# tyb311/TCCT

Measured on AMD Instinct MI355X. Metric: OCT B-scans/sec fwd+bwd(+clip+AdamW), stc_tt bs=8 1x800x1100, higher is better.
Workload: dtype bf16; 1 GPU; stc_tt --los=di bs=8/GPU 1x800x1100 (net tensors 3x800x1104); global_batch=8, parallelism=dp1, ranks=1, grad_allreduce=none, slowest_step=136

## Files before the change

### tcct_amd/csrc/pw_mfma.hip

```cpp
#include "common.h"
#include "c3_geom.h"
#include <cstdlib>

typedef __attribute__((ext_vector_type(8))) __bf16 bf16x8;
typedef __attribute__((ext_vector_type(16))) float f32x16;
typedef __attribute__((ext_vector_type(4))) short s16x4;
typedef __attribute__((ext_vector_type(8))) short s16x8;

#define PWB 256

__device__ __forceinline__ void st_out4(bf16* p, float a, float b, float c, float d) {
    uint2 o; o.x = pack_bf16x2(a, b); o.y = pack_bf16x2(c, d);
    *reinterpret_cast<uint2*>(p) = o;
}
__device__ __forceinline__ void st_out4(float* p, float a, float b, float c, float d) {
    *reinterpret_cast<float4*>(p) = make_float4(a, b, c, d);
}


struct PwUp { const float* p; int uH, uW, Ho, Wo; float sh, sw; uint32_t m_howo, m_wo; };
struct PwSplit { const bf16* x2; int K1; void* y2; int N1; const bf16* res; const float* rscale; int64_t per_sample; bf16* yplain; C3Geom c3; PwUp up; };
template <int NT, typename Tout, bool STATS, bool AFF, bool C3 = false>
__global__ void __launch_bounds__(PWB, 2)
k_pw_fwd(const bf16* __restrict__ x, const float* __restrict__ w, const float* __restrict__ bias, Tout* __restrict__ y,
// ... 315 lines not shown
    const int64_t M = (int64_t)B * Ho * Wo;
    TCCT_CHECK(M < (1ll << 31), "pw_fwd_f32_upadd: %lld pixels exceed the 32-bit index arithmetic", (long long)M);
    PwSplit sp{nullptr, 0, nullptr, 0, nullptr, nullptr, 1, nullptr};
    sp.up = PwUp{up, uH, uW, Ho, Wo, Ho > 1 ? (float)(uH - 1) / (float)(Ho - 1) : 0.f, Wo > 1 ? (float)(uW - 1) / (float)(Wo - 1) : 0.f,
                 (uint32_t)((1ull << 32) / (uint64_t)(Ho * Wo)), (uint32_t)((1ull << 32) / (uint64_t)Wo)};
    return pw_fwd_impl(x, w, bias, y, M, K, N, 0, TCCT_F32, nullptr, 0, stream, nullptr, 0, 0, sp);
}
extern "C" int tcct_pw_dgrad_split2(const void* dy, const float* w, void* dx1, void* dx2, int K1, int64_t M, int Nout, int K,
                                    tcct_stream_t stream) {
    TCCT_CHECK(dx2 != nullptr, "pw_dgrad_split2: dx2 is NULL");
    return pw_fwd_impl(dy, w, nullptr, dx1, M, Nout, K, 1, TCCT_BF16, nullptr, 0, stream, nullptr, 0, 0, PwSplit{nullptr, 0, dx2, K1, nullptr, nullptr, 1, nullptr});
}
extern "C" int tcct_pw_fwd_residual(const void* x, const float* w, const float* bias, const void* res, const float* scale,
                                    int64_t per_sample, void* y, void* y_plain, int64_t M, int K, int N, tcct_stream_t stream) {
    TCCT_CHECK(res != nullptr && N % 32 == 0 && per_sample >= 1, "pw_fwd_residual: needs res, N %% 32 == 0, per_sample >= 1");
    return pw_fwd_impl(x, w, bias, y, M, K, N, 0, TCCT_BF16, nullptr, 0, stream, nullptr, 0, 0,
                       PwSplit{nullptr, 0, nullptr, 0, (const bf16*)res, scale, per_sample, (bf16*)y_plain});
}
extern "C" int tcct_pw_dgrad_residual(const void* dy, const float* w, const void* res, void* dx_sum, void* dx_plain, int64_t M, int Nout,
                                      int K, tcct_stream_t stream) {
    TCCT_CHECK(res != nullptr && K % 32 == 0, "pw_dgrad_residual: needs res, K %% 32 == 0");
    return pw_fwd_impl(dy, w, nullptr, dx_sum, M, Nout, K, 1, TCCT_BF16, nullptr, 0, stream, nullptr, 0, 0,
                       PwSplit{nullptr, 0, nullptr, 0, (const bf16*)res, nullptr, 1, (bf16*)dx_plain});
}
extern "C" int tcct_pw_fwd_affine(const void* x, const float* w, const float* bias, void* y, int64_t M, int K, int N, const float* ab,
                                  int pre_act, int post_act, int out_dtype, tcct_stream_t stream) {
    return pw_fwd_impl(x, w, bias, y, M, K, N, 0, out_dtype, nullptr, 0, stream, ab, pre_act, post_act);
}
extern "C" int tcct_pw_fwd_affine_residual(const void* x, const float* w, const float* bias, const float* ab, const void* res, void* y, int64_t M, int K, int N,
                                           tcct_stream_t stream) {
    TCCT_CHECK(res != nullptr && pw_fwd2_aff_ok(M, K, N, false, true), "pw_fwd_affine_residual: K=%d N=%d unsupported (64, 96 or 128 square) or res NULL", K, N);
    return pw_fwd2_launch(x, nullptr, w, bias, y, M, K, N, nullptr, 0, stream, pw_res_affine((const bf16*)res, nullptr, ab, TCCT_ACT_NONE));
}
extern "C" int tcct_pw_fwd_xaff_affine_residual(const void* y_prev, const float* ab_prev, const float* w, const float* bias, const float* ab, const void* res, void* y,
                                                int64_t M, int K, int N, tcct_stream_t stream) {
    TCCT_CHECK(y_prev && ab_prev && res != nullptr && pw_fwd2_aff_ok(M, K, N, false, true), "pw_fwd_xaff_affine_residual: K=%d N=%d unsupported (64, 96 or 128 square) or NULL argument", K, N);
    PwFwd2Mode md;
    md.xap = TCCT_ACT_HSWISH;
    return pw_fwd2_launch(y_prev, nullptr, w, bias, y, M, K, N, nullptr, 0, stream, pw_res_affine((const bf16*)res, ab_prev, ab, TCCT_ACT_NONE), md);
}
extern "C" int tcct_pw_fwd_cat2_affine(const void* x1, const void* x2, const float* w, const float* bias, const float* ab, int post_act, void* y, int64_t M, int K, int N,
                                       tcct_stream_t stream) {
    TCCT_CHECK(x2 != nullptr && pw_fwd2_aff_ok(M, K, N, true, false), "pw_fwd_cat2_affine: K=%d N=%d unsupported (64 + 64 -> 96)", K, N);
    return pw_fwd2_launch(x1, x2, w, bias, y, M, K, N, nullptr, 0, stream, pw_res_affine(nullptr, nullptr, ab, post_act));
}
static int pw_fwd_impl(const void* x, const float* w, const float* bias, void* y, int64_t M, int K, int N, int transposed,
                       int out_dtype, double* stats, int stat_pre, tcct_stream_t stream, const float* aff, int aff_pre, int aff_post, PwSplit sp) {
    if (!transposed && out_dtype == TCCT_BF16 && (aff || aff_post) && !aff_pre && !stats && !sp.y2 && !sp.yplain && !sp.rscale && pw_fwd2_enabled()
        && pw_fwd2_aff_ok(M, K, N, sp.x2 != nullptr, sp.res != nullptr) && (!sp.x2 || sp.K1 == 64))
        return pw_fwd2_launch(x, sp.x2, w, bias, y, M, K, N, nullptr, 0, stream, pw_res_affine(sp.res, nullptr, aff, aff_post));
    if (!transposed && out_dtype == TCCT_BF16 && !aff && !aff_pre && !aff_post && !sp.y2 && pw_fwd2_enabled()
        && pw_fwd2_ok(M, K, N, sp.K1, sp.x2 != nullptr) && (!stats || N <= 128) && !(sp.res && (sp.x2 || stats)))
        return pw_fwd2_launch(x, sp.x2, w, bias, y, M, K, N, stats, stat_pre, stream, pw_res_train(sp.res, sp.rscale, sp.per_sample, sp.yplain));
    if (sp.x2) TCCT_CHECK(sp.K1 % 32 == 0 && sp.K1 > 0 && sp.K1 < K, "pw_fwd_cat2: K1=%d must be a multiple of 32 inside (0, K)", sp.K1);
    if (sp.y2) TCCT_CHECK(sp.N1 % 32 == 0 && sp.N1 > 0 && sp.N1 < N && N % 32 == 0 && out_dtype == TCCT_BF16, "pw_dgrad_split2: N1=%d must be a multiple of 32 inside (0, N), bf16 output", sp.N1);
    TCCT_CHECK(K % 32 == 0 && K >= 32 && K <= 512, "pw_fwd: K=%d must be a multiple of 32 (<=512)", K);
    TCCT_CHECK(N >= 1 && N <= 1024, "pw_fwd: N=%d", N);
    const int ntiles = (N + 31) / 32;
    int NT = ntiles <= 5 ? ntiles : (ntiles % 5 == 0 ? 5 : (ntiles % 4 == 0 ? 4 : (ntiles % 3 == 0 ? 3 : (ntiles % 2 == 0 ? 2 : 1))));
    const int64_t mblocks = ((M + 31) / 32 + 3) / 4;
    while (NT > 1 && mblocks * ((ntiles + NT - 1) / NT) < 512) {
        int nn = NT - 1;
        while (nn > 1 && ntiles % nn != 0) --nn;
        NT = nn;
    }
    if (stats && NT > 4) NT = 1;
    const int gy = (ntiles + NT - 1) / NT;
    size_t lds = (((size_t)NT * 32 * (2 * K + 16) + 15) & ~(size_t)15) + 4 * 2560 + (size_t)NT * 32 * 4;
    TCCT_CHECK(lds <= 160 * 1024, "pw_fwd: weights need %zu B of LDS", lds);
    const int64_t mtiles = (M + 31) / 32;
    int64_t gx = (mtiles + 3) / 4;
    int per_cu = (int)((160 * 1024) / lds);
    if (per_cu > 4) per_cu = 4;
    if (per_cu < 1) per_cu = 1;
    const int cap = 256 * per_cu;
    if (gx > cap) gx = cap;
    hipStream_t st = (hipStream_t)stream;
#define PW_GO(NTV, TO, ST, AF) tcct_launch<k_pw_fwd<NTV, TO, ST, AF>, 160 * 1024>(dim3((unsigned)gx, gy), dim3(PWB), lds, st, (const bf16*)x, w, bias, (TO*)y, M, K, N, transposed, \
                                                                                stats, stats ? stat_pre : 0, aff, aff_pre, aff_post, sp)
#define PW_NT4(TO, ST, AF) case 1: PW_GO(1, TO, ST, AF); break; case 2: PW_GO(2, TO, ST, AF); break; case 3: PW_GO(3, TO, ST, AF); break; case 4: PW_GO(4, TO, ST, AF); break
    bool hit = true;
    if (aff || aff_pre || aff_post || sp.res) {
        TCCT_CHECK(out_dtype == TCCT_BF16 && !stats, "pw_fwd_affine: bf16 output only");
        switch (NT) { PW_NT4(bf16, false, true); case 5: PW_GO(5, bf16, false, true); break; default: hit = false; }
    }
    else if (stats) switch (NT) { PW_NT4(bf16, true, false); default: hit = false; }
    else if (out_dtype == TCCT_BF16) switch (NT) { PW_NT4(bf16, false, false); case 5: PW_GO(5, bf16, false, false); break; default: hit = false; }
    else if (out_dtype == TCCT_F32) switch (NT) { PW_NT4(float, false, false); case 5: PW_GO(5, float, false, false); break; default: hit = false; }
    else { tcct_set_error("pw_fwd: bad out dtype"); return -1; }
#undef PW_NT4
#undef PW_GO
    TCCT_CHECK(hit, "pw_fwd: no kernel for %d N-tiles per block (stats %d)", NT, stats != nullptr);
    TCCT_LAUNCH_OK();
}

extern "C" int tcct_c3_fwd(const void* x4, const float* w, const float* bias, void* y, int B, int H, int W, int stride, double* stats,
                           int stat_pre, const float* ab, int pre_act, int post_act, tcct_stream_t stream) {
    TCCT_CHECK(stride == 1 || stride == 2, "c3_fwd: stride %d", stride);
    TCCT_CHECK(!(stats && (ab || pre_act || post_act)), "c3_fwd: fused statistics and the inference epilogue exclude each other");
    TCCT_CHECK(!stats || stat_pre == 0, "c3_fwd: the fused statistics are those of the raw output (both first layers feed a BatchNorm directly)");
    const int Ho = (H - 1) / stride + 1, Wo = (W - 1) / stride + 1;
    const int64_t M = (int64_t)B * Ho * Wo, inb = (int64_t)B * H * W * 8;
    TCCT_CHECK(M > 0 && M < (1ll << 31) - 64 && inb < (1ll << 31), "c3_fwd: image too large for 32-bit pixel offsets (B=%d H=%d W=%d)", B, H, W);
    const int tpr = (Wo + 31) / 32;
    auto magic = [](uint32_t d) { return d == 1 ? 0xffffffffu : (uint32_t)((1ull << 32) / d); };
    PwSplit sp{nullptr, 0, nullptr, 0, nullptr, nullptr, 1, nullptr,
               C3Geom{H, W, Ho, Wo, stride, (uint32_t)inb, tpr, magic((uint32_t)tpr), magic((uint32_t)Ho), magic((uint32_t)(Ho * Wo)), magic((uint32_t)Wo)}};
    const size_t lds = (((size_t)32 * (2 * 48 + 16) + 15) & ~(size_t)15) + 4 * 2560 + 32 * 4;
    const int64_t mtiles = (int64_t)B * Ho * tpr;
    int64_t gx = (mtiles + 3) / 4;
    if (gx > 256 * 4) gx = 256 * 4;
    hipStream_t st = (hipStream_t)stream;
    if (stats)
        hipLaunchKernelGGL((k_pw_fwd<1, bf16, true, false, true>), dim3((unsigned)gx, 1), dim3(PWB), lds, st, (const bf16*)x4, w, bias, (bf16*)y, M, 48, 32, 0,
                           stats, stat_pre, nullptr, 0, 0, sp);
    else if (ab || pre_act || post_act)
        hipLaunchKernelGGL((k_pw_fwd<1, bf16, false, true, true>), dim3((unsigned)gx, 1), dim3(PWB), lds, st, (const bf16*)x4, w, bias, (bf16*)y, M, 48, 32, 0,
                           nullptr, 0, ab, pre_act, post_act, sp);
    else
        hipLaunchKernelGGL((k_pw_fwd<1, bf16, false, false, true>), dim3((unsigned)gx, 1), dim3(PWB), lds, st, (const bf16*)x4, w, bias, (bf16*)y, M, 48, 32, 0,
                           nullptr, 0, nullptr, 0, 0, sp);
    TCCT_LAUNCH_OK();
}

__device__ __forceinline__ bf16x8 tr_load8g(const unsigned char* base, int stride, int P, int chan0, int lane) {
    const int i = lane & 15, q = i >> 2, pp = i & 3, g = lane >> 4;
    const int hh = g >> 1, cb = g & 1;
    const unsigned char* a0 = base + (P + 8 * hh + q) * stride + (chan0 + 16 * cb + 4 * pp) * 2;
    s16x4 lo = __builtin_amdgcn_ds_read_tr16_b64_v4i16((__attribute__((address_space(3))) s16x4*)a0);
    s16x4 hi = __builtin_amdgcn_ds_read_tr16_b64_v4i16((__attribute__((address_space(3))) s16x4*)(a0 + 4 * stride));
    s16x8 v = __builtin_shufflevector(lo, hi, 0, 1, 2, 3, 4, 5, 6, 7);
    return __builtin_bit_cast(bf16x8, v);
}

#define PW_P 128
#define PW_XS 4
#define PW_DS 10
template <int NT, int KTB, bool C3 = false>
__global__ void __launch_bounds__(PWB, 2)
k_pw_wgrad(const bf16* __restrict__ x, const bf16* __restrict__ dy, float* __restrict__ dw, float* __restrict__ dbias, int64_t M,
           int K, int N, int SX, int SD, const bf16* __restrict__ x2, int K1, int64_t ldy, C3Geom g3 = C3Geom{0, 0, 0, 0, 0, 0u, 0, 0u, 0u, 0u, 0u}) {
    extern __shared__ __attribute__((aligned(16))) unsigned char smem[];
    unsigned char* sX = smem;
    unsigned char* sD = smem + PW_P * SX;
    const int tid = threadIdx.x, lane = tid & 63, wave = tid >> 6;
    const int r = lane & 31, hh = lane >> 5;
    const int ci_base = blockIdx.y * KTB * 32;
    const bf16* xsrc = (x2 && ci_base >= K1) ? x2 + (ci_base - K1) : x + ci_base;
    const int ldx = x2 ? (ci_base >= K1 ? K - K1 : K1) : K;
    const int xc = KTB * 4, dc = N >> 3;
    f32x16 acc[NT][KTB];
#pragma unroll
    for (int a = 0; a < NT; ++a)
#pragma unroll
        for (int b = 0; b < KTB; ++b)
#pragma unroll
            for (int k = 0; k < 16; ++k) acc[a][b][k] = 0.f;
    float bsum[NT];
#pragma unroll
    for (int a = 0; a < NT; ++a) bsum[a] = 0.f;
    constexpr int DSN = C3 ? 2 : PW_DS;
    static_assert(!C3 || (NT == 1 && KTB == 2), "C3 weight gradient: 32 outputs, 48 (-> 64) patch elements");
    int xsl[PW_XS], dsl[DSN];
#pragma unroll
    for (int j = 0; j < PW_XS; ++j) {
        int i = tid + j * PWB; xsl[j] = i < PW_P * xc ? ((i / xc) << 8) | (i % xc) : -1;
        if (C3) xsl[j] = j < 3 ? ((tid & 127) << 8) | (2 * j + (tid >> 7)) : -1;
    }
    const __amdgpu_buffer_rsrc_t c3r = __builtin_amdgcn_make_buffer_rsrc((void*)x, 0, C3 ? g3.bytes : 0u, 0x00020000);
    const __amdgpu_buffer_rsrc_t c3d = __builtin_amdgcn_make_buffer_rsrc((void*)dy, 0, C3 ? (uint32_t)(M * 64) : 0u, 0x00020000);
#pragma unroll
    for (int j = 0; j < DSN; ++j) { int i = tid + j * PWB; dsl[j] = i < PW_P * dc ? ((i / dc) << 8) | (i % dc) : -1; }
    uint4 px[PW_XS], pd[DSN];
    auto prefetch = [&](int64_t tile) {
        const int64_t m0 = tile * PW_P;
        if (C3) {
            const uint32_t mm = (uint32_t)(m0 + (tid & 127));
            const bool in = m0 + (tid & 127) < M;
            const uint32_t n_ = udiv_m(mm, (uint32_t)(g3.Ho * g3.Wo), g3.m_howo), rem = mm - n_ * (uint32_t)(g3.Ho * g3.Wo);
            const uint32_t oy = udiv_m(rem, (uint32_t)g3.Wo, g3.m_wo), ox = rem - oy * (uint32_t)g3.Wo;
            const int iy0 = (int)oy * g3.stride - 1, ix0 = (int)ox * g3.stride - 1;
            const int hi = tid >> 7;
            const int pa = ix0 + 2 * hi, pb = ix0 + 1;
            const bool va = in & ((unsigned)pa < (unsigned)g3.W), vb = in & (hi == 0) & ((unsigned)pb < (unsigned)g3.W);
            const int base = ((int)(n_ * (uint32_t)g3.H) + iy0) * g3.W;
#pragma unroll
            for (int ky = 0; ky < 3; ++ky) {
                const bool rv = (unsigned)(iy0 + ky) < (unsigned)g3.H;
                const uint32_t offa = (va & rv) ? (uint32_t)(base + ky * g3.W + pa) * 8u : 0x80000000u;
                const uint32_t offb = (vb & rv) ? (uint32_t)(base + ky * g3.W + pb) * 8u : 0x80000000u;
                const uint2 ta = __builtin_bit_cast(uint2, __builtin_amdgcn_raw_buffer_load_b64(c3r, offa, 0, 0));
                const uint2 tb = __builtin_bit_cast(uint2, __builtin_amdgcn_raw_buffer_load_b64(c3r, offb, 0, 0));
                px[ky] = make_uint4(ta.x, ta.y, tb.x, tb.y);
            }
        } else
#pragma unroll
        for (int j = 0; j < PW_XS; ++j) {
            px[j] = make_uint4(0, 0, 0, 0);
            if (xsl[j] >= 0 && m0 + (xsl[j] >> 8) < M)
                px[j] = *reinterpret_cast<const uint4*>(xsrc + (m0 + (xsl[j] >> 8)) * ldx + (xsl[j] & 255) * 8);
        }
#pragma unroll
        for (int j = 0; j < DSN; ++j) {
            if (C3) {
                pd[j] = __builtin_bit_cast(uint4, __builtin_amdgcn_raw_buffer_load_b128(c3d, (uint32_t)m0 * 64u + (uint32_t)(tid + j * PWB) * 16u, 0, 0));
                continue;
            }
            pd[j] = make_uint4(0, 0, 0, 0);
            if (dsl[j] >= 0 && m0 + (dsl[j] >> 8) < M)
                pd[j] = *reinterpret_cast<const uint4*>(dy + (m0 + (dsl[j] >> 8)) * ldy + (dsl[j] & 255) * 8);
        }
    };
    const int li = lane & 15, lq = li >> 2, lpp = li & 3, lg = lane >> 4;
    const int lrow = 8 * (lg >> 1) + lq, lcol = (16 * (lg & 1) + 4 * lpp) * 2;
    const unsigned char* lbX = sX + lrow * SX + lcol;
    const unsigned char* lbD = sD + lrow * SD + lcol;
    auto tr2 = [&](const unsigned char* p, int stride) {
        s16x4 lo = __builtin_amdgcn_ds_read_tr16_b64_v4i16((__attribute__((address_space(3))) s16x4*)p);
        s16x4 hi = __builtin_amdgcn_ds_read_tr16_b64_v4i16((__attribute__((address_space(3))) s16x4*)(p + 4 * stride));
        s16x8 v = __builtin_shufflevector(lo, hi, 0, 1, 2, 3, 4, 5, 6, 7);
        return __builtin_bit_cast(bf16x8, v);
    };
    struct WF { bf16x8 a[NT], b[KTB]; };
    auto load_chunk = [&](WF& f, int ch) {
#pragma unroll
        for (int ct = 0; ct < NT; ++ct) f.a[ct] = tr2(lbD + ch * 16 * SD + 64 * ct, SD);
#pragma unroll
        for (int kt = 0; kt < KTB; ++kt) f.b[kt] = tr2(lbX + ch * 16 * SX + 64 * kt, SX);
    };
    auto mma_chunk = [&](const WF& f) {
        if (blockIdx.y == 0) {
#pragma unroll
            for (int ct = 0; ct < NT; ++ct)
#pragma unroll
                for (int j = 0; j < 8; ++j) bsum[ct] += (float)f.a[ct][j];
        }
#pragma unroll
        for (int kt = 0; kt < KTB; ++kt)
#pragma unroll
            for (int ct = 0; ct < NT; ++ct) acc[ct][kt] = __builtin_amdgcn_mfma_f32_32x32x16_bf16(f.a[ct], f.b[kt], acc[ct][kt], 0, 0, 0);
    };
    const int64_t tiles = (M + PW_P - 1) / PW_P;
    int64_t tile = blockIdx.x;
    if (C3)
        for (int i = tid; i < PW_P * 2; i += PWB) *reinterpret_cast<uint4*>(sX + (i >> 1) * SX + (6 + (i & 1)) * 16) = make_uint4(0, 0, 0, 0);
    if (tile < tiles) prefetch(tile);
    for (; tile < tiles; tile += gridDim.x) {
        __syncthreads();
        if (C3) {
#pragma unroll
            for (int j = 0; j < 3; ++j)
                if (xsl[j] >= 0) *reinterpret_cast<uint4*>(sX + (tid & 127) * SX + (xsl[j] & 255) * 16) = px[j];
        } else
#pragma unroll
        for (int j = 0; j < PW_XS; ++j)
            if (xsl[j] >= 0) *reinterpret_cast<uint4*>(sX + (xsl[j] >> 8) * SX + (xsl[j] & 255) * 16) = px[j];
#pragma unroll
        for (int j = 0; j < DSN; ++j)
            if (dsl[j] >= 0) *reinterpret_cast<uint4*>(sD + (dsl[j] >> 8) * SD + (dsl[j] & 255) * 16) = pd[j];
        __syncthreads();
        if (C3 || tile + gridDim.x < tiles) prefetch(tile + gridDim.x);
        WF f0, f1;
        load_chunk(f0, wave);
        load_chunk(f1, wave + 4);
        __builtin_amdgcn_sched_barrier(0);
        mma_chunk(f0);
        mma_chunk(f1);
        __builtin_amdgcn_sched_barrier(0);
    }
    __syncthreads();
    float* red = reinterpret_cast<float*>(smem);
    for (int turn = 0; turn < 4; ++turn) {
        if (wave == turn) {
#pragma unroll
            for (int ct = 0; ct < NT; ++ct)
#pragma unroll
                for (int kt = 0; kt < KTB; ++kt)
#pragma unroll
                    for (int k = 0; k < 16; ++k) {
                        const int co = ct * 32 + (k & 3) + 8 * (k >> 2) + 4 * hh;
                        float* dst = &red[co * (KTB * 32) + kt * 32 + r];
                        *dst = turn == 0 ? acc[ct][kt][k] : *dst + acc[ct][kt][k];
                    }
        }
        __syncthreads();
    }
    for (int i = tid; i < NT * 32 * KTB * 32; i += PWB) {
        const int co = i / (KTB * 32), cl = i - co * (KTB * 32);
        if (C3) {
            if (cl < 48 && ((cl >> 2) & 3) < 3 && (cl & 3) < 3) atomicAdd(&dw[co * 27 + (cl & 3) * 9 + (cl >> 4) * 3 + ((cl >> 2) & 3)], red[i]);
        }
        else
        if (co < N && ci_base + cl < K) atomicAdd(&dw[(int64_t)co * K + ci_base + cl], red[i]);
    }
    if (dbias && blockIdx.y == 0) {
#pragma unroll
        for (int ct = 0; ct < NT; ++ct) {
            float s = bsum[ct] + __shfl_xor(bsum[ct], 32, 64);
            if (lane < 32 && ct * 32 + r < N) atomicAdd(&dbias[ct * 32 + r], s);
        }
    }
}

static int pw_wgrad_impl(const void* x, const void* x2, int K1, const void* dy, float* dw, float* dbias, int64_t M, int K, int N, tcct_stream_t stream,
                         int64_t ldy);
extern "C" int tcct_pw_wgrad(const void* x, const void* dy, float* dw, float* dbias, int64_t M, int K, int N, tcct_stream_t stream) {
    return pw_wgrad_impl(x, nullptr, 0, dy, dw, dbias, M, K, N, stream, 0);
}
extern "C" int tcct_pw_wgrad_cat2(const void* x1, const void* x2, int K1, const void* dy, float* dw, float* dbias, int64_t M, int K, int N,
                                  tcct_stream_t stream) {
    TCCT_CHECK(x2 != nullptr && K1 % 32 == 0 && K1 > 0 && K1 < K, "pw_wgrad_cat2: K1=%d must be a multiple of 32 inside (0, K)", K1);
    return pw_wgrad_impl(x1, x2, K1, dy, dw, dbias, M, K, N, stream, 0);
}
extern "C" int tcct_pw_wgrad_strided(const void* x, const void* dy, int64_t ldy, float* dw, float* dbias, int64_t M, int K, int N,
                                     tcct_stream_t stream) {
    return pw_wgrad_impl(x, nullptr, 0, dy, dw, dbias, M, K, N, stream, ldy);
}
static int pw_wgrad_impl(const void* x, const void* x2, int K1, const void* dy, float* dw, float* dbias, int64_t M, int K, int N, tcct_stream_t stream,
                         int64_t ldy) {
    if (ldy == 0) ldy = N;
    TCCT_CHECK(ldy >= N && ldy % 8 == 0, "pw_wgrad: ldy=%lld must be a multiple of 8 and >= N=%d", (long long)ldy, N);
    TCCT_CHECK(K % 32 == 0 && N % 32 == 0 && K >= 32 && N >= 32 && N <= 160 && K <= 1024, "pw_wgrad: unsupported K=%d N=%d", K, N);
    hipStream_t st = (hipStream_t)stream;
    if (!tcct_skip_zero_fill() && hipMemsetAsync(dw, 0, sizeof(float) * (size_t)N * K, st) != hipSuccess) { tcct_set_error("pw_wgrad: memset failed"); return -2; }
    if (dbias && !tcct_skip_zero_fill() && hipMemsetAsync(dbias, 0, sizeof(float) * N, st) != hipSuccess) { tcct_set_error("pw_wgrad: memset failed"); return -2; }
    const int NT = N / 32, ktiles = K / 32;
    const int KTB = (ktiles % 2 == 0 && NT <= 2) ? 2 : 1;
    const int gy = ktiles / KTB;
    TCCT_CHECK(!x2 || K1 % (KTB * 32) == 0, "pw_wgrad_cat2: K1=%d must be a multiple of %d for this shape", K1, KTB * 32);
    const int SX = KTB == 1 ? 64 : 192;
    const int SD = 2 * N + ((NT & 1) ? 0 : 64);
    size_t lds = (size_t)PW_P * (SX + SD);
    size_t red = (size_t)NT * 32 * KTB * 32 * 4;
    if (red > lds) lds = red;
    const int64_t tiles = (M + PW_P - 1) / PW_P;
    int per_cu = (int)((160 * 1024) / (lds + 512));
    if (per_cu > 2) per_cu = 2;
    if (per_cu < 1) per_cu = 1;
    int gx = 256 * per_cu / gy;
    if (gx < 64) gx = 64;
    if (tiles <= 1024) { int small = 128 / gy; if (small < 16) small = 16; if (gx > small) gx = small; }
    if (gx > tiles) gx = (int)tiles;
    if (gx < 1) gx = 1;
#define WL(NTV, KV) tcct_launch<k_pw_wgrad<NTV, KV>, 160 * 1024>(dim3(gx, gy), dim3(PWB), lds, st, (const bf16*)x, (const bf16*)dy, dw, dbias, M, K, N, SX, SD, (const bf16*)x2, K1, ldy, C3Geom{})
    if (KTB == 2) { switch (NT) { case 1: WL(1, 2); break; default: WL(2, 2); break; } }
    else { switch (NT) { case 1: WL(1, 1); break; case 2: WL(2, 1); break; case 3: WL(3, 1); break; case 4: WL(4, 1); break; default: WL(5, 1); break; } }
#undef WL
    TCCT_LAUNCH_OK();
}


extern "C" int tcct_c3_wgrad(const void* x4, const void* dy, float* dw, float* dbias, int B, int H, int W, int stride, tcct_stream_t stream) {
    TCCT_CHECK(stride == 1 || stride == 2, "c3_wgrad: stride %d", stride);
    const int Ho = (H - 1) / stride + 1, Wo = (W - 1) / stride + 1;
    const int64_t M = (int64_t)B * Ho * Wo, inb = (int64_t)B * H * W * 8;
    TCCT_CHECK(M > 0 && M * 64 < (1ll << 31) && inb < (1ll << 31), "c3_wgrad: image too large for 32-bit byte offsets (B=%d H=%d W=%d)", B, H, W);
    hipStream_t st = (hipStream_t)stream;
    if (!tcct_skip_zero_fill() && hipMemsetAsync(dw, 0, sizeof(float) * 32 * 27, st) != hipSuccess) { tcct_set_error("c3_wgrad: memset failed"); return -2; }
    if (dbias && !tcct_skip_zero_fill() && hipMemsetAsync(dbias, 0, sizeof(float) * 32, st) != hipSuccess) { tcct_set_error("c3_wgrad: memset failed"); return -2; }
    const int SX = 192, SD = 64;
    const size_t lds = (size_t)PW_P * (SX + SD);
    const int64_t tiles = (M + PW_P - 1) / PW_P;
    int gx = (int)(tiles / 48 < 256 ? 256 : (tiles / 48 > 1024 ? 1024 : tiles / 48));
    if (gx > tiles) gx = (int)tiles;
    auto magic = [](uint32_t d) { return d == 1 ? 0xffffffffu : (uint32_t)((1ull << 32) / d); };
    hipLaunchKernelGGL((k_pw_wgrad<1, 2, true>), dim3(gx, 1), dim3(PWB), lds, st, (const bf16*)x4, (const bf16*)dy, dw, dbias, M, 64, 32, SX, SD,
                       (const bf16*)nullptr, 0, (int64_t)32,
                       C3Geom{H, W, Ho, Wo, stride, (uint32_t)inb, (Wo + 31) / 32, magic((uint32_t)((Wo + 31) / 32)), magic((uint32_t)Ho), magic((uint32_t)(Ho * Wo)), magic((uint32_t)Wo)});
    TCCT_LAUNCH_OK();
}


#define PB_P 128

__device__ __forceinline__ u32x4 gelu8(u32x4 v) {
    u32x4 o;
#pragma unroll
    for (int k = 0; k < 4; ++k)
        o[k] = pack_bf16x2(act_c<TCCT_ACT_GELU>(__uint_as_float(v[k] << 16)), act_c<TCCT_ACT_GELU>(__uint_as_float(v[k] & 0xffff0000u)));
    return o;
}
__device__ __forceinline__ float gelu_grad1(float x) { float c, p; gauss_cdf_pdf(x, c, p); return c + x * p; }
template <int KIND> __device__ __forceinline__ u32x4 affine8(u32x4 v, const float* __restrict__ a, const float* __restrict__ b) {
    const float4 a0 = *reinterpret_cast<const float4*>(a), a1 = *reinterpret_cast<const float4*>(a + 4);
    const float4 b0 = *reinterpret_cast<const float4*>(b), b1 = *reinterpret_cast<const float4*>(b + 4);
    const float aa[8] = {a0.x, a0.y, a0.z, a0.w, a1.x, a1.y, a1.z, a1.w}, bb[8] = {b0.x, b0.y, b0.z, b0.w, b1.x, b1.y, b1.z, b1.w};
    u32x4 o;
#pragma unroll
    for (int k = 0; k < 4; ++k)
        o[k] = pack_bf16x2(act_c<KIND>(aa[2 * k] * __uint_as_float(v[k] << 16) + bb[2 * k]),
                           act_c<KIND>(aa[2 * k + 1] * __uint_as_float(v[k] & 0xffff0000u) + bb[2 * k + 1]));
    return o;
}
struct PwBnBwd { const bf16* y; const float* coef; const bf16* yprev; const float* abprev; double* sums_prev;
                 const double* sums; int raw; const float* mean_rstd; const float* ab; float* dgamma; float* dbeta; };
template <int KIND> __device__ __forceinline__ float pw_act_grad(float u) {
    if (KIND == TCCT_ACT_HSWISH) return u < -3.f ? 0.f : (u <= 3.f ? (2.f * u + 3.f) * (1.f / 6.f) : 1.f);
    return 1.f;
}
template <int NT, int KT, bool SPLIT = false, int BNP = -1, int REDP = -1, bool GX = false, int XAP = -1, bool LNB = false, bool DY2 = false>
__global__ void __launch_bounds__(PWB, 2)
k_pw_bwd(const bf16* __restrict__ x, const bf16* __restrict__ dy, const float* __restrict__ w, const bf16* __restrict__ res,
         bf16* __restrict__ dx, bf16* __restrict__ dx_plain, float* __restrict__ dw, float* __restrict__ dbias, int64_t M, PwBnBwd bn) {
    constexpr int K = 32 * KT, N = 32 * NT;
    constexpr bool BN = BNP >= 0, RED = REDP >= 0;
    constexpr int SX = 64 * KT + ((KT & 1) ? 0 : 64), SD = 64 * NT + ((NT & 1) ? 0 : 64);
    constexpr int SW = 2 * N + 16;
    constexpr int XS = K / 16, DS = N / 16;
    extern __shared__ __attribute__((aligned(16))) unsigned char smem[];
    unsigned char* sX = smem;
    unsigned char* sD = sX + PB_P * SX;
    unsigned char* sW = sD + PB_P * SD;
    unsigned char* sS = sW + ((K * SW + 15) & ~15);
    float* sC = reinterpret_cast<float*>(sS + 4 * 2560);
    float* sP = sC + (BN ? 5 * N : 0);
    const int tid = threadIdx.x, lane = tid & 63, wave = tid >> 6;
    const int r = lane & 31, hh = lane >> 5;
    for (int i = tid; i < N * K; i += PWB) {
        const int n = i / K, k = i - n * K;
        *reinterpret_cast<bf16*>(sW + k * SW + n * 2) = __float2bfloat16(w[i]);
    }
    if (BN) {
        if (bn.coef) { for (int i = tid; i < 5 * N; i += PWB) sC[i] = bn.coef[i]; }
        else if (tid < N) {
            const int c = tid;
            const double mu = bn.mean_rstd[c], rs = bn.mean_rstd[N + c];
            const double S1 = bn.sums[c];
            const double S2 = bn.raw ? (bn.sums[N + c] - mu * S1) * rs : bn.sums[N + c];
            if (blockIdx.x == 0) { bn.dbeta[c] = (float)S1; bn.dgamma[c] = (float)S2; }
            const double a = bn.ab[c], s1 = S1 / (double)M, s2 = S2 / (double)M;
            sC[c] = (float)a; sC[N + c] = (float)(-a * s2 * rs); sC[2 * N + c] = (float)(a * (s2 * rs * mu - s1));
            sC[3 * N + c] = bn.ab[c]; sC[4 * N + c] = bn.ab[N + c];
        }
    }
    if (RED || XAP >= 0) for (int i = tid; i < 2 * (SPLIT ? K / 2 : K); i += PWB) sP[i] = bn.abprev[i];
    if (LNB) for (int i = tid; i < K; i += PWB) sP[i] = bn.abprev[i];
    constexpr int RKT = LNB ? KT : (RED ? (SPLIT ? KT / 2 : KT) : 1);
    float rs[RKT][8], rq[RKT][8];
#pragma unroll
    for (int a = 0; a < RKT; ++a)
#pragma unroll
        for (int k = 0; k < 8; ++k) rs[a][k] = rq[a][k] = 0.f;
    f32x16 accw[(NT * KT + 3) / 4];
#pragma unroll
    for (int a = 0; a < (NT * KT + 3) / 4; ++a)
#pragma unroll
        for (int k = 0; k < 16; ++k) accw[a][k] = 0.f;
    float bsum[(NT * KT + 3) / 4];
#pragma unroll
    for (int a = 0; a < (NT * KT + 3) / 4; ++a) bsum[a] = 0.f;
    const int64_t tiles = (M + PB_P - 1) / PB_P;
    constexpr int KS = SPLIT ? K / 2 : K;
    const uint32_t xbytes = (uint32_t)(M * KS * 2), dbytes = (uint32_t)(M * N * 2);
    const __amdgpu_buffer_rsrc_t rx = __builtin_amdgcn_make_buffer_rsrc((void*)x, 0, xbytes, 0x00020000);
    const __amdgpu_buffer_rsrc_t rd = __builtin_amdgcn_make_buffer_rsrc((void*)dy, 0, dbytes, 0x00020000);
    const __amdgpu_buffer_rsrc_t rr = __builtin_amdgcn_make_buffer_rsrc((void*)(res ? res : x), 0, xbytes, 0x00020000);
    const __amdgpu_buffer_rsrc_t ro = __builtin_amdgcn_make_buffer_rsrc((void*)dx, 0, xbytes, 0x00020000);
    const __amdgpu_buffer_rsrc_t rp = __builtin_amdgcn_make_buffer_rsrc((void*)(dx_plain ? dx_plain : dx), 0, xbytes, 0x00020000);
    const __amdgpu_buffer_rsrc_t ry = __builtin_amdgcn_make_buffer_rsrc((void*)((BN || DY2) ? bn.y : dy), 0, dbytes, 0x00020000);
    const __amdgpu_buffer_rsrc_t ryp = __builtin_amdgcn_make_buffer_rsrc((void*)((RED || LNB) ? bn.yprev : x), 0, xbytes, 0x00020000);
    u32x4 px[XS], pd[DS], py[(BN || DY2) ? DS : 1];
    auto prefetch = [&](int64_t tile) {
        const uint32_t bx = (uint32_t)(tile * PB_P * KS * 2), bd = (uint32_t)(tile * PB_P * N * 2);
#pragma unroll
        for (int j = 0; j < XS; ++j) {
            if (SPLIT && j >= XS / 2) px[j] = __builtin_amdgcn_raw_buffer_load_b128(rr, bx + (uint32_t)(tid + (j - XS / 2) * PWB) * 16u, 0, 0);
            else px[j] = __builtin_amdgcn_raw_buffer_load_b128(rx, bx + (uint32_t)(tid + j * PWB) * 16u, 0, 0);
        }
#pragma unroll
        for (int j = 0; j < DS; ++j) pd[j] = __builtin_amdgcn_raw_buffer_load_b128(rd, bd + (uint32_t)(tid + j * PWB) * 16u, 0, 0);
        if (BN || DY2) {
#pragma unroll
            for (int j = 0; j < DS; ++j) py[j] = __builtin_amdgcn_raw_buffer_load_b128(ry, bd + (uint32_t)(tid + j * PWB) * 16u, 0, 0);
        }
    };
    auto stage_x1 = [&](int j, u32x4 xv_) {
        const int jj = (SPLIT && j >= XS / 2) ? j - XS / 2 : j;
        const int q = tid + jj * PWB, p = q / (KS / 8), c = q - p * (KS / 8);
        if (GX) xv_ = gelu8(xv_);
        if (XAP >= 0) xv_ = affine8<XAP < 0 ? 0 : XAP>(xv_, sP + c * 8, sP + KS + c * 8);
        *reinterpret_cast<u32x4*>(sX + p * SX + ((SPLIT && j >= XS / 2) ? KS * 2 : 0) + c * 16) = xv_;
    };
    auto stage_d = [&](int64_t tile) {
#pragma unroll
        for (int j = 0; j < DS; ++j) {
            const int q = tid + j * PWB, p = q / (N / 8), c = q - p * (N / 8);
            u32x4 v = pd[j];
            if (DY2) {
#pragma unroll
                for (int k = 0; k < 4; ++k)
                    v[k] = pack_bf16x2(__uint_as_float(pd[j][k] << 16) + __uint_as_float(py[j][k] << 16),
                                       __uint_as_float(pd[j][k] & 0xffff0000u) + __uint_as_float(py[j][k] & 0xffff0000u));
            }
            if (BN) {
                const bool live = tile * PB_P + p < M;
                const float* cc = sC + c * 8;
#pragma unroll
                for (int h = 0; h < 2; ++h) {
                    const float4 c1 = *reinterpret_cast<const float4*>(cc + 4 * h), c2 = *reinterpret_cast<const float4*>(cc + N + 4 * h);
                    const float4 c3 = *reinterpret_cast<const float4*>(cc + 2 * N + 4 * h);
                    float4 ca = c1, cb = c1;
                    if (BNP != TCCT_ACT_NONE) { ca = *reinterpret_cast<const float4*>(cc + 3 * N + 4 * h); cb = *reinterpret_cast<const float4*>(cc + 4 * N + 4 * h); }
                    const float k1[4] = {c1.x, c1.y, c1.z, c1.w}, k2[4] = {c2.x, c2.y, c2.z, c2.w}, k3[4] = {c3.x, c3.y, c3.z, c3.w};
                    const float ka[4] = {ca.x, ca.y, ca.z, ca.w}, kb[4] = {cb.x, cb.y, cb.z, cb.w};
#pragma unroll
                    for (int e2 = 0; e2 < 2; ++e2) {
                        const uint32_t gz = pd[j][2 * h + e2], gy = py[j][2 * h + e2];
                        float z0 = __uint_as_float(gz << 16), z1 = __uint_as_float(gz & 0xffff0000u);
                        const float y0 = __uint_as_float(gy << 16), y1 = __uint_as_float(gy & 0xffff0000u);
                        if (BNP != TCCT_ACT_NONE) {
                            z0 *= pw_act_grad<BNP>(ka[2 * e2] * y0 + kb[2 * e2]);
                            z1 *= pw_act_grad<BNP>(ka[2 * e2 + 1] * y1 + kb[2 * e2 + 1]);
                        }
                        const float o0 = k1[2 * e2] * z0 + k2[2 * e2] * y0 + k3[2 * e2];
                        const float o1 = k1[2 * e2 + 1] * z1 + k2[2 * e2 + 1] * y1 + k3[2 * e2 + 1];
                        v[2 * h + e2] = live ? pack_bf16x2(o0, o1) : 0u;
                    }
                }
            }
            *reinterpret_cast<u32x4*>(sD + p * SD + c * 16) = v;
        }
    };
    auto stage = [&](int64_t tile) {
#pragma unroll
        for (int j = 0; j < XS; ++j) stage_x1(j, px[j]);
        stage_d(tile);
    };
    const int li = lane & 15, lq = li >> 2, lpp = li & 3, lg = lane >> 4;
    const int lrow = 8 * (lg >> 1) + lq, lcol = (16 * (lg & 1) + 4 * lpp) * 2;
    const unsigned char* lbX = sX + lrow * SX + lcol;
    const unsigned char* lbD = sD + lrow * SD + lcol;
    auto tr2 = [&](const unsigned char* p, int stride) {
        s16x4 lo = __builtin_amdgcn_ds_read_tr16_b64_v4i16((__attribute__((address_space(3))) s16x4*)p);
        s16x4 hi = __builtin_amdgcn_ds_read_tr16_b64_v4i16((__attribute__((address_space(3))) s16x4*)(p + 4 * stride));
        s16x8 v = __builtin_shufflevector(lo, hi, 0, 1, 2, 3, 4, 5, 6, 7);
        return __builtin_bit_cast(bf16x8, v);
    };
    int64_t tile = blockIdx.x;
    if (tile < tiles) {
        prefetch(tile);
        __syncthreads();
        stage(tile);
        prefetch(tile + gridDim.x);
    }
    __syncthreads();
    for (; tile < tiles; tile += gridDim.x) {
        u32x4 xq[GX ? KT : 1][2];
        if (GX) {
            const int64_t m0q = tile * PB_P + 32 * wave;
#pragma unroll
            for (int kt = 0; kt < KT; ++kt)
#pragma unroll
                for (int h2 = 0; h2 < 2; ++h2) {
                    const int64_t mm = m0q + (lane >> 2) + 16 * h2;
                    xq[kt][h2] = __builtin_amdgcn_raw_buffer_load_b128(rx, mm < M ? (uint32_t)((mm * K + kt * 32 + (lane & 3) * 8) * 2) : 0x80000000u, 0, 0);
                }
        }
        u32x4 tq[LNB ? KT : 1][2];
        float tmean[2] = {0.f, 0.f}, trstd[2] = {0.f, 0.f};
        if (LNB) {
            const int64_t m0q = tile * PB_P + 32 * wave;
#pragma unroll
            for (int h2 = 0; h2 < 2; ++h2) {
                const int64_t mm = m0q + (lane >> 2) + 16 * h2;
#pragma unroll
                for (int kt = 0; kt < KT; ++kt)
                    tq[kt][h2] = __builtin_amdgcn_raw_buffer_load_b128(ryp, mm < M ? (uint32_t)((mm * K + kt * 32 + (lane & 3) * 8) * 2) : 0x80000000u, 0, 0);
                if (mm < M) { const float2 mr = *reinterpret_cast<const float2*>(bn.mean_rstd + 2 * mm); tmean[h2] = mr.x; trstd[h2] = mr.y; }
            }
        }
        u32x4 yq[RKT][2];
        if (RED) {
            const int64_t m0q = tile * PB_P + 32 * wave;
#pragma unroll
            for (int kt = 0; kt < RKT; ++kt)
#pragma unroll
                for (int h2 = 0; h2 < 2; ++h2) {
                    const int64_t mm = m0q + (lane >> 2) + 16 * h2;
                    yq[kt][h2] = __builtin_amdgcn_raw_buffer_load_b128(ryp, mm < M ? (uint32_t)((mm * KS + kt * 32 + (lane & 3) * 8) * 2) : 0x80000000u, 0, 0);
                }
        }
#pragma unroll
        for (int a = 0; a < (NT * KT + 3) / 4; ++a) {
            const int ti = wave + 4 * a;
            if (ti < NT * KT) {
                const int ct = ti / KT, kt = ti - ct * KT;
#pragma unroll
                for (int ch = 0; ch < 8; ++ch) {
                    const bf16x8 fa = tr2(lbD + ch * 16 * SD + 64 * ct, SD);
                    const bf16x8 fb = tr2(lbX + ch * 16 * SX + 64 * kt, SX);
                    if (kt == 0) {
#pragma unroll
                        for (int j = 0; j < 8; ++j) bsum[a] += (float)fa[j];
                    }
                    accw[a] = __builtin_amdgcn_mfma_f32_32x32x16_bf16(fa, fb, accw[a], 0, 0, 0);
                }
            }
        }
        f32x16 accd[KT];
#pragma unroll
        for (int kt = 0; kt < KT; ++kt)
#pragma unroll
            for (int k = 0; k < 16; ++k) accd[kt][k] = 0.f;
        const unsigned char* bB = sD + (32 * wave + r) * SD + hh * 16;
#pragma unroll
        for (int st = 0; st < 2 * NT; ++st) {
            const bf16x8 fb = *reinterpret_cast<const bf16x8*>(bB + st * 32);
#pragma unroll
            for (int kt = 0; kt < KT; ++kt) {
                const bf16x8 fa = *reinterpret_cast<const bf16x8*>(sW + (kt * 32 + r) * SW + st * 32 + hh * 16);
                accd[kt] = __builtin_amdgcn_mfma_f32_32x32x16_bf16(fa, fb, accd[kt], 0, 0, 0);
            }
        }
        __syncthreads();
        if ((GX || XAP >= 0) && !SPLIT) {
            const bool do_stage = tile + (int64_t)gridDim.x < tiles;
            const int64_t tp = tile + 2 * (int64_t)gridDim.x;
            const uint32_t bx = (uint32_t)(tp * PB_P * KS * 2), bd = (uint32_t)(tp * PB_P * N * 2);
#pragma unroll
            for (int j = 0; j < XS; ++j) {
                const u32x4 xv_ = px[j];
                px[j] = __builtin_amdgcn_raw_buffer_load_b128(rx, bx + (uint32_t)(tid + j * PWB) * 16u, 0, 0);
                if (do_stage) stage_x1(j, xv_);
            }
            if (do_stage) stage_d(tile + (int64_t)gridDim.x);
#pragma unroll
            for (int j = 0; j < DS; ++j) pd[j] = __builtin_amdgcn_raw_buffer_load_b128(rd, bd + (uint32_t)(tid + j * PWB) * 16u, 0, 0);
            if (BN) {
#pragma unroll
                for (int j = 0; j < DS; ++j) py[j] = __builtin_amdgcn_raw_buffer_load_b128(ry, bd + (uint32_t)(tid + j * PWB) * 16u, 0, 0);
            }
// ... 785 lines not shown
```

Before: 417.8 B-scans/s.

## Add tile-owning pointwise weight-gradient kernel with register accumulators

Adds a new weight-gradient kernel in which each wave owns several 32x32 output tiles and accumulates them in registers across a persistent loop over M tiles. Each block covers a wider K slab, so the dy tile is reused across more input-channel tiles and the grid has fewer y-blocks. The LDS reduction and the per-block atomic pass of the old kernel are replaced by direct stores or one atomic per owned element. It also adds register prefetch of the next tile and a lookup table of supported (NT, KT) shapes. The costs are higher register pressure and lower parallelism when M is small, and the old path still runs for shapes not in the table.

Result: no change. 418.6 B-scans/s, median of 6 (+0.2%).

```diff
diff --git a/tcct_amd/csrc/pw_mfma.hip b/tcct_amd/csrc/pw_mfma.hip
--- a/tcct_amd/csrc/pw_mfma.hip
+++ b/tcct_amd/csrc/pw_mfma.hip
@@ -641,6 +641,129 @@
     }
 }
 
+#define PO_P 64
+template <int NT, int KT>
+__global__ void __launch_bounds__(PWB, 2)
+k_pw_wgrad_own(const bf16* __restrict__ x, const bf16* __restrict__ dy, float* __restrict__ dw, float* __restrict__ dbias, int64_t M, int K,
+               const bf16* __restrict__ x2, int K1, int64_t ldy) {
+    constexpr int SX = 64 * KT + ((KT & 1) ? 0 : 64), SD = 64 * NT + ((NT & 1) ? 0 : 64);
+    constexpr int XC = 4 * KT, DC = 4 * NT;
+    constexpr int OWN = (NT * KT + 3) / 4;
+    static_assert(OWN <= 8, "k_pw_wgrad_own: more than 8 owned tiles per wave do not fit the register file without scratch");
+    extern __shared__ __attribute__((aligned(16))) unsigned char smem[];
+    unsigned char* sX = smem;
+    unsigned char* sD = smem + PO_P * SX;
+    const int tid = threadIdx.x, lane = tid & 63, wave = __builtin_amdgcn_readfirstlane(tid >> 6);
+    const int r = lane & 31, hh = lane >> 5;
+    const int ci_base = blockIdx.y * KT * 32;
+    f32x16 acc[OWN];
+#pragma unroll
+    for (int a = 0; a < OWN; ++a)
+#pragma unroll
+        for (int k = 0; k < 16; ++k) acc[a][k] = 0.f;
+    float bsum[OWN];
+#pragma unroll
+    for (int a = 0; a < OWN; ++a) bsum[a] = 0.f;
+    u32x4 px[KT], pd[NT];
+    auto prefetch = [&](int64_t tile) {
+        const int64_t m0 = tile * PO_P;
+#pragma unroll
+        for (int j = 0; j < KT; ++j) {
+            const int q = tid + j * PWB, p = q / XC, ch = ci_base + (q - p * XC) * 8;
+            const int64_t m = m0 + p < M ? m0 + p : M - 1;
+            const bf16* src = ch < K1 ? x + m * K1 + ch : x2 + m * (K - K1) + (ch - K1);
+            px[j] = *reinterpret_cast<const u32x4*>(src);
+        }
+#pragma unroll
+        for (int j = 0; j < NT; ++j) {
+            const int q = tid + j * PWB, p = q / DC, c = q - p * DC;
+            const int64_t m = m0 + p < M ? m0 + p : M - 1;
+            pd[j] = *reinterpret_cast<const u32x4*>(dy + m * ldy + c * 8);
+        }
+    };
+    auto stage = [&](int64_t tile) {
+        const int64_t m0 = tile * PO_P;
+        const u32x4 zero = {0u, 0u, 0u, 0u};
+#pragma unroll
+        for (int j = 0; j < KT; ++j) {
+            const int q = tid + j * PWB, p = q / XC, c = q - p * XC;
+            *reinterpret_cast<u32x4*>(sX + p * SX + c * 16) = m0 + p < M ? px[j] : zero;
+        }
+#pragma unroll
+        for (int j = 0; j < NT; ++j) {
+            const int q = tid + j * PWB, p = q / DC, c = q - p * DC;
+            *reinterpret_cast<u32x4*>(sD + p * SD + c * 16) = m0 + p < M ? pd[j] : zero;
+        }
+    };
+    const int li = lane & 15, lq = li >> 2, lpp = li & 3, lg = lane >> 4;
+    const int lrow = 8 * (lg >> 1) + lq, lcol = (16 * (lg & 1) + 4 * lpp) * 2;
+    const unsigned char* lbX = sX + lrow * SX + lcol;
+    const unsigned char* lbD = sD + lrow * SD + lcol;
+    auto tr2 = [&](const unsigned char* p, int stride) {
+        s16x4 lo = __builtin_amdgcn_ds_read_tr16_b64_v4i16((__attribute__((address_space(3))) s16x4*)p);
+        s16x4 hi = __builtin_amdgcn_ds_read_tr16_b64_v4i16((__attribute__((address_space(3))) s16x4*)(p + 4 * stride));
+        s16x8 v = __builtin_shufflevector(lo, hi, 0, 1, 2, 3, 4, 5, 6, 7);
+        return __builtin_bit_cast(bf16x8, v);
+    };
+    const int64_t tiles = (M + PO_P - 1) / PO_P;
+    int64_t tile = blockIdx.x;
+    if (tile < tiles) prefetch(tile);
+    for (; tile < tiles; tile += gridDim.x) {
+        __syncthreads();
+        stage(tile);
+        __syncthreads();
+        if (tile + gridDim.x < tiles) prefetch(tile + gridDim.x);
+#pragma unroll
+        for (int a = 0; a < OWN; ++a) {
+            const int ti = wave + 4 * a;
+            if (ti < NT * KT) {
+                const int ct = ti / KT, kt = ti - ct * KT;
+#pragma unroll
+                for (int ch = 0; ch < PO_P / 16; ++ch) {
+                    const bf16x8 fa = tr2(lbD + ch * 16 * SD + 64 * ct, SD);
+                    const bf16x8 fb = tr2(lbX + ch * 16 * SX + 64 * kt, SX);
+                    if (kt == 0 && blockIdx.y == 0) {
+#pragma unroll
+                        for (int j = 0; j < 8; ++j) bsum[a] += (float)fa[j];
+                    }
+                    acc[a] = __builtin_amdgcn_mfma_f32_32x32x16_bf16(fa, fb, acc[a], 0, 0, 0);
+                }
+            }
+        }
+    }
+    const bool single = gridDim.x == 1;
+#pragma unroll
+    for (int a = 0; a < OWN; ++a) {
+        const int ti = wave + 4 * a;
+        if (ti < NT * KT) {
+            const int ct = ti / KT, kt = ti - ct * KT;
+#pragma unroll
+            for (int k = 0; k < 16; ++k) {
+                const int co = ct * 32 + (k & 3) + 8 * (k >> 2) + 4 * hh;
+                float* dst = &dw[(int64_t)co * K + ci_base + kt * 32 + r];
+                if (single) *dst = acc[a][k]; else atomicAdd(dst, acc[a][k]);
+            }
+            if (dbias && kt == 0 && blockIdx.y == 0) {
+                const float sb = bsum[a] + __shfl_xor(bsum[a], 32, 64);
+                if (lane < 32) { if (single) dbias[ct * 32 + r] = sb; else atomicAdd(&dbias[ct * 32 + r], sb); }
+            }
+        }
+    }
+}
+
+typedef void (*PwWgradOwnLaunch)(dim3, dim3, size_t, hipStream_t, const bf16*, const bf16*, float*, float*, int64_t, int, const bf16*, int, int64_t);
+struct PwWgradOwnRow { int nt, kt; PwWgradOwnLaunch launch; };
+#define PWO_ROW(NT, KT) {NT, KT, tcct_launch<k_pw_wgrad_own<NT, KT>, 160 * 1024>}
+static const PwWgradOwnRow pw_wgrad_own_table[] = { PWO_ROW(5, 5), PWO_ROW(5, 4), PWO_ROW(4, 6), PWO_ROW(4, 4), PWO_ROW(3, 3), PWO_ROW(1, 5) };
+#undef PWO_ROW
+static const PwWgradOwnRow* pw_wgrad_own_find(int nt, int ktiles) {
+    const PwWgradOwnRow* best = nullptr;
+    for (const PwWgradOwnRow& r : pw_wgrad_own_table)
+        if (r.nt == nt && ktiles % r.kt == 0 && (!best || r.kt > best->kt)) best = &r;
+    return best;
+}
+#define PW_OWN_MIN_TILES 4
+
 static int pw_wgrad_impl(const void* x, const void* x2, int K1, const void* dy, float* dw, float* dbias, int64_t M, int K, int N, tcct_stream_t stream,
                          int64_t ldy);
 extern "C" int tcct_pw_wgrad(const void* x, const void* dy, float* dw, float* dbias, int64_t M, int K, int N, tcct_stream_t stream) {
@@ -666,6 +789,17 @@
     const int NT = N / 32, ktiles = K / 32;
     const int KTB = (ktiles % 2 == 0 && NT <= 2) ? 2 : 1;
     const int gy = ktiles / KTB;
+    const PwWgradOwnRow* own = M > 0 ? pw_wgrad_own_find(NT, ktiles) : nullptr;
+    if (own && ktiles / own->kt < gy) {
+        const int oy = ktiles / own->kt;
+        const int SXo = 64 * own->kt + ((own->kt & 1) ? 0 : 64), SDo = 64 * NT + ((NT & 1) ? 0 : 64);
+        const int64_t otiles = (M + PO_P - 1) / PO_P;
+        int64_t ox = otiles / PW_OWN_MIN_TILES;
+        if (ox > 512 / oy) ox = 512 / oy;
+        if (ox < 1) ox = 1;
+        own->launch(dim3((unsigned)ox, oy), dim3(PWB), (size_t)PO_P * (SXo + SDo), st, (const bf16*)x, (const bf16*)dy, dw, dbias, M, K, (const bf16*)x2, x2 ? K1 : K, ldy);
+        TCCT_LAUNCH_OK();
+    }
     TCCT_CHECK(!x2 || K1 % (KTB * 32) == 0, "pw_wgrad_cat2: K1=%d must be a multiple of %d for this shape", K1, KTB * 32);
     const int SX = KTB == 1 ? 64 : 192;
     const int SD = 2 * N + ((NT & 1) ? 0 : 64);
```
